# sipposip/pr-disagg-radar-gan

Measured on AMD Instinct MI355X. Metric: cWGAN-GP train samples/sec, 24x16x16 tiles, bs=256, higher is better.
Workload: dtype f32; 1 GPU; ndomain=16, 24h, bs=256 fp32, 1 critic step + 1 gen step (BASELINE configs[1]); batch_per_gpu=256, global_batch=256, n_critic=1, parallelism=dp1, world=1, rccl_ranks_seen=1, weights=random init (RandomNormal 0.02 / glorot_uniform), dropout 0.25 active

## Files before the change

include/rdgan.h:

```cpp
#ifndef RDGAN_H
#define RDGAN_H
#include <stdint.h>
#ifdef __cplusplus
extern "C" {
#endif

typedef struct rdgan_handle rdgan_handle;

#define RDGAN_LATENT_DIM 100
#define RDGAN_NHOURS 24
#define RDGAN_LOSS_SLOTS 8

int rdgan_create(rdgan_handle** out, int ndomain, int n_cond_channels, int max_batch);
void rdgan_destroy(rdgan_handle* h);
const char* rdgan_last_error(const rdgan_handle* h);
long rdgan_gen_param_count(const rdgan_handle* h);
long rdgan_critic_param_count(const rdgan_handle* h);
long rdgan_workspace_bytes(const rdgan_handle* h);

int rdgan_gen_forward(rdgan_handle* h, const float* gen_params, const float* z, const float* cond,
                      float* out, int B, void* stream);

int rdgan_check_numerics(rdgan_handle* h, void* stream);

int rdgan_critic_forward(rdgan_handle* h, const float* critic_params, const float* sample,
                         const float* cond, float* out, int B, uint64_t seed, void* stream);

int rdgan_critic_grad(rdgan_handle* h, const float* critic_params, const float* gen_params,
                      const float* x_real, const float* cond, const float* z, uint64_t seed,
                      float* grad_out, int B, void* stream);

int rdgan_critic_grad_after(rdgan_handle* h, const float* critic_params, const float* gen_params,
                            const float* x_real, const float* cond, const float* z, uint64_t seed,
                            float* grad_out, int B, void* critic_ready_event, void* stream);

int rdgan_gen_grad(rdgan_handle* h, const float* critic_params, const float* gen_params,
                   const float* z, const float* cond, uint64_t seed, float* grad_out, int B,
                   void* stream);

int rdgan_gen_grad_after(rdgan_handle* h, const float* critic_params, const float* gen_params,
                         const float* z, const float* cond, uint64_t seed, float* grad_out, int B,
                         void* critic_ready_event, void* stream);

int rdgan_adam(float* params, const float* grad, float* v, long n, int t, float lr, float beta2,
               float eps, float grad_scale, void* stream);

int rdgan_set_weight_versions(rdgan_handle* h, uint64_t gen_version, uint64_t critic_version);
int rdgan_form_builds(const rdgan_handle* h, long* gen_builds, long* critic_builds);

int rdgan_gen_param_layout(const rdgan_handle* h, long* offsets, long* sizes);
int rdgan_critic_param_layout(const rdgan_handle* h, long* offsets, long* sizes);

int rdgan_set_option(rdgan_handle* h, const char* name, int value);

enum {
  RDGAN_TAG_GCONV_FWD = 0,
  RDGAN_TAG_GCONV_DGRAD = 1,
// ... 87 lines not shown
```

pr_disagg_radar_gan_amd/_lib.py:

```python
import ctypes
import os

_HERE = os.path.dirname(os.path.abspath(__file__))
LIB_PATH = os.path.join(_HERE, "librdgan_hip.so")

c_f32p = ctypes.c_void_p
c_stream = ctypes.c_void_p

class LaunchStat(ctypes.Structure):
    _fields_ = [("plan", ctypes.c_int), ("kind", ctypes.c_int), ("batch", ctypes.c_int), ("launches", ctypes.c_int),
                ("gflop", ctypes.c_double), ("ms", ctypes.c_double), ("name", ctypes.c_char * 48), ("kernel", ctypes.c_char * 48)]


SIGNATURES = {
    "rdgan_create": (ctypes.c_int, [ctypes.POINTER(ctypes.c_void_p), ctypes.c_int, ctypes.c_int, ctypes.c_int]),
    "rdgan_destroy": (None, [ctypes.c_void_p]),
    "rdgan_last_error": (ctypes.c_char_p, [ctypes.c_void_p]),
    "rdgan_gen_param_count": (ctypes.c_long, [ctypes.c_void_p]),
    "rdgan_critic_param_count": (ctypes.c_long, [ctypes.c_void_p]),
    "rdgan_workspace_bytes": (ctypes.c_long, [ctypes.c_void_p]),
    "rdgan_gen_forward": (ctypes.c_int, [ctypes.c_void_p, c_f32p, c_f32p, c_f32p, c_f32p, ctypes.c_int, c_stream]),
    "rdgan_check_numerics": (ctypes.c_int, [ctypes.c_void_p, c_stream]),
    "rdgan_critic_forward": (ctypes.c_int, [ctypes.c_void_p, c_f32p, c_f32p, c_f32p, c_f32p, ctypes.c_int,
                                            ctypes.c_uint64, c_stream]),
    "rdgan_critic_grad": (ctypes.c_int, [ctypes.c_void_p, c_f32p, c_f32p, c_f32p, c_f32p, c_f32p, ctypes.c_uint64,
                                         c_f32p, ctypes.c_int, c_stream]),
    "rdgan_gen_grad": (ctypes.c_int, [ctypes.c_void_p, c_f32p, c_f32p, c_f32p, c_f32p, ctypes.c_uint64, c_f32p,
                                      ctypes.c_int, c_stream]),
    "rdgan_critic_grad_after": (ctypes.c_int, [ctypes.c_void_p, c_f32p, c_f32p, c_f32p, c_f32p, c_f32p, ctypes.c_uint64,
                                               c_f32p, ctypes.c_int, ctypes.c_void_p, c_stream]),
    "rdgan_gen_grad_after": (ctypes.c_int, [ctypes.c_void_p, c_f32p, c_f32p, c_f32p, c_f32p, ctypes.c_uint64, c_f32p,
                                            ctypes.c_int, ctypes.c_void_p, c_stream]),
    "rdgan_adam": (ctypes.c_int, [c_f32p, c_f32p, c_f32p, ctypes.c_long, ctypes.c_int, ctypes.c_float, ctypes.c_float,
                                  ctypes.c_float, ctypes.c_float, c_stream]),
    "rdgan_set_weight_versions": (ctypes.c_int, [ctypes.c_void_p, ctypes.c_uint64, ctypes.c_uint64]),
    "rdgan_form_builds": (ctypes.c_int, [ctypes.c_void_p, ctypes.POINTER(ctypes.c_long), ctypes.POINTER(ctypes.c_long)]),
    "rdgan_gen_param_layout": (ctypes.c_int, [ctypes.c_void_p, ctypes.POINTER(ctypes.c_long), ctypes.POINTER(ctypes.c_long)]),
    "rdgan_critic_param_layout": (ctypes.c_int, [ctypes.c_void_p, ctypes.POINTER(ctypes.c_long), ctypes.POINTER(ctypes.c_long)]),
    "rdgan_set_option": (ctypes.c_int, [ctypes.c_void_p, ctypes.c_char_p, ctypes.c_int]),
    "rdgan_profile": (ctypes.c_int, [ctypes.c_void_p, ctypes.c_uint]),
    "rdgan_flop_count": (ctypes.c_int, [ctypes.c_void_p, ctypes.POINTER(ctypes.c_double), ctypes.c_int]),
    "rdgan_profile_read": (ctypes.c_int, [ctypes.c_void_p, ctypes.c_int, ctypes.POINTER(ctypes.c_double),
                                          ctypes.POINTER(ctypes.c_long)]),
    "rdgan_profile_launches": (ctypes.c_int, [ctypes.c_void_p, ctypes.c_int]),
    "rdgan_launch_table": (ctypes.c_int, [ctypes.c_void_p, ctypes.POINTER(LaunchStat), ctypes.c_int, ctypes.POINTER(ctypes.c_int)]),
    "rdgan_data_gather": (ctypes.c_int, [c_f32p, ctypes.c_int, ctypes.c_int, ctypes.c_int, ctypes.c_void_p, ctypes.c_int,
                                         ctypes.c_int, ctypes.c_float, c_f32p, c_f32p, ctypes.c_void_p, c_stream]),
    "rdgan_data_valid_tiles": (ctypes.c_int, [c_f32p, ctypes.c_int, ctypes.c_int, ctypes.c_int, ctypes.c_int, ctypes.c_int,
                                              ctypes.c_float, ctypes.c_int, ctypes.c_void_p, c_stream]),
    "rdgan_crps_ensemble": (ctypes.c_int, [c_f32p, c_f32p, c_f32p, c_f32p, ctypes.c_int, ctypes.c_long, c_stream]),
    "rdgan_spectra_bins": (ctypes.c_int, [ctypes.c_int]),
    "rdgan_radial_spectra": (ctypes.c_int, [c_f32p, c_f32p, ctypes.c_long, ctypes.c_int, ctypes.c_int, c_stream]),
    "rdgan_lsd_workspace_bytes": (ctypes.c_long, [ctypes.c_long, ctypes.c_long]),
# ... 74 lines not shown
```

pr_disagg_radar_gan_amd/csrc/rdgan_api.hip:

```cpp
#include <hip/hip_runtime.h>
#include <stdio.h>
#include <string.h>
#include <math.h>
#include <string>
#include <vector>
#include <algorithm>
#include <unordered_set>

#include "../../include/rdgan.h"
#include "rdgan_plan.h"
#include "rdgan_hostplan.h"
#include "rdgan_rng.h"
#include "rdgan_gemm.hip.h"
#include "rdgan_gemm_ws.hip.h"
#include "rdgan_gemm_ws16.hip.h"
#include "rdgan_gemm_f16.hip.h"
#include "rdgan_upconv16.hip.h"
#include "rdgan_upconv16b.hip.h"
#include "rdgan_upconv16t.hip.h"
#include "rdgan_elem.hip.h"
#include "rdgan_data.hip.h"
#include "rdgan_edge.hip.h"
#include "rdgan_d2slab16.hip.h"
#include "rdgan_d2fwd16.hip.h"
// ... 70 lines not shown
  int collapse = 1;
  int tapgather = 1;
  int ws_ksplit = 1;
  int wave_spec = 1;
  int resident = 1;
  int edge_kernels = 1;
  int sample_offset = 0;
  float* g9b_tmp;
  float* gp_part;
  float* dw6_part;
  int side_on = 1;
  int split3 = 0;
  int dense_slices = 0;
  uint64_t gver_in = 0, cver_in = 0;
  const float* gcache_ptr = nullptr; uint64_t gcache_ver = 0; int gcache_cfg = -1;
  const float* ccache_ptr = nullptr; uint64_t ccache_ver = 0; int ccache_cfg = -1;
  long form_builds[2] = {0, 0};
  int keep_gates = 0;
  void* gate_keep[5] = {nullptr, nullptr, nullptr, nullptr, nullptr};
  int gate_keep_B = 0;
  hipStream_t side = nullptr;
  hipEvent_t ev_fork = nullptr, ev_join = nullptr, ev_cw = nullptr, ev_g[4] = {nullptr, nullptr, nullptr, nullptr};
  int* d_flag;
  std::unordered_set<const void*> lds_attr_done;
  int prof_launches = 0;
  std::vector<RdLaunchRec> launch_recs;
  size_t launch_used = 0;
  char cur_kernel[48] = {0};
  double flops_acc = 0;
  unsigned prof_mask = 0;
  std::vector<hipEvent_t> ev_start[RDGAN_NUM_TAGS], ev_stop[RDGAN_NUM_TAGS];
  size_t ev_used[RDGAN_NUM_TAGS] = {0};
};

#define RD_CHECK(h, call)                                                        \
  do {                                                                           \
    hipError_t e_ = (call);                                                      \
    if (e_ != hipSuccess) {                                                      \
      char b_[512];                                                              \
      snprintf(b_, sizeof b_, "%s:%d %s -> %s", __FILE__, __LINE__, #call, hipGetErrorString(e_)); \
      if (h) (h)->err = b_;                                                      \
      return (int)e_;                                                            \
    }                                                                            \
  } while (0)
#define RD_TRY(expr)            \
  do {                          \
// ... 665 lines not shown
    carve(h->h1, MB * h->gpix[1] * 256); carve(h->r1, MB * h->gpix[1]);
    carve(h->h2, MB * h->gpix[2] * 128); carve(h->r2, MB * h->gpix[2]);
    carve(h->h3, MB * h->gpix[3] * 64); carve(h->r3, MB * h->gpix[3]);
    carve(h->P9, MB * h->gpix[3] * 32);
    carve(h->fake, MB * h->gpix[3]);
    carve(h->dl, MB * h->gpix[3]);
    carve(h->gh3, MB * h->gpix[3] * 64);
    carve(h->gup3, MB * h->gpix[3] * 128);
    carve(h->dy2, MB * h->gpix[2] * 128);
    carve(h->gup2, MB * h->gpix[2] * 256);
    carve(h->dy1, MB * h->gpix[1] * 256);
    carve(h->gup1, MB * h->gpix[1] * 256);
    carve(h->ga0, MB * h->gpix[0] * 256);
    carve(h->cin, NB * h->dL[0] * h->CP);
    h->dh[0] = nullptr; h->du[0] = nullptr;
    for (int l = 1; l <= 4; ++l) { carve(h->dh[l], NB * h->dL[l] * dch[l]); carve(h->du[l], NB * h->dL[l] * dch[l]); }
    carve(h->v, NB);
    carve(h->P1, MB * h->dL[1] * h->ldp1);
    carve(h->g0, MB * h->dL[0]);
    carve(h->gpv, MB);
    carve(h->wpartial, h->wpartial_cap);
    carve(h->cpartial, h->cpartial_cap);
    carve(h->kpartial, h->kpartial_cap);
    h->DWT[0] = h->DWT[1] = nullptr;
    for (int l = 2; l <= 4; ++l) carve(h->DWT[l], 27L * dch[l - 1] * dch[l]);
    carve(h->W1T, 64 * h->ldp1);
    carve(h->W1P, 27L * h->CP * 64); carve(h->dW1P, 27L * h->CP * 64);
    h->GWT[0] = nullptr;
    for (int l = 1; l <= 3; ++l) carve(h->GWT[l], 27L * gch[l - 1] * gch[l]);
    carve(h->W9T, 64 * 32);
    h->GWC[0] = h->GWD[0] = nullptr;
    for (int l = 1; l <= 3; ++l) { carve(h->GWC[l], 64L * gch[l - 1] * gch[l]); carve(h->GWD[l], 64L * gch[l - 1] * gch[l]); }
    carve(h->dWc, 64L * 256 * 256);
    {
      size_t ne = 0, ns = 0;
      for (int l = 1; l <= 3; ++l) {
        const int* sd = h->gdim[l - 1];
        ne = std::max(ne, (size_t)(sd[0] + 1) * sd[1] * sd[2] * gch[l - 1]);
        ns = std::max(ns, (size_t)sd[0] * 4 * sd[1] * sd[2] * gch[l]);
      }
      h->fE[0] = h->fU[0] = nullptr;
      for (int l = 1; l <= 3; ++l) {
        const int* sd = h->gdim[l - 1];
        carve(h->fE[l], MB * (size_t)(sd[0] + 1) * sd[1] * sd[2] * gch[l - 1]);
        carve(h->fU[l], 48L * gch[l - 1] * gch[l]);
      }
// ... 12 lines not shown
          carve(p, 27L * dch[l - 1] * dch[l] / 2 + 8); h->bWB[l] = p;
        }
        h->bG1F[0] = nullptr;
        for (int l = 1; l <= 3; ++l) { carve(p, 32L * gch[l - 1] * gch[l] + 8); h->bG1F[l] = p; }
        carve(p, 32L * 256 * 256 + 8); h->bG1B = p;
        h->fWF[0] = h->fWF[1] = h->fWB[0] = h->fWB[1] = h->fG1F[0] = nullptr;
        for (int l = 2; l <= 4; ++l) {
          carve(p, 27L * dch[l - 1] * dch[l] / 2 + 8); h->fWF[l] = p;
          carve(p, 27L * dch[l - 1] * dch[l] / 2 + 8); h->fWB[l] = p;
        }
        for (int l = 1; l <= 3; ++l) { carve(p, 32L * gch[l - 1] * gch[l] + 8); h->fG1F[l] = p; }
        carve(p, 32L * 256 * 256 + 8); h->fG1B = p;
        carve(p, 32L * h->ldp1 + 8); h->bW1B = p;
        carve(p, 64L * 8 * 2 * 64 * 4 + 8); h->bW3I = p;
        carve(p, 64L * 8 * 2 * 64 * 4 + 8); h->bW3T = p;
        carve(p, 4L * 64 * 4 + 8); h->bW9I = p;
        carve(p, (long)RD_UP2_KSTEPS * 4 * 64 * 4 + 8); h->bW2I = p;
        carve(p, (long)RD_D2S_KSTEPS * 2 * 64 * 4 + 8); h->bW2S = p;
        if (nd % 16 == 0) { carve(p, NB * h->dL[1] * 4 + 8); if (pass == 1) h->g1bits = (unsigned char*)p; }
        carve(p, (long)RD_D2F_KSTEPS * 4 * 64 * 4 + 8); h->bW2F = p;
      }
      carve(h->fdU, 48L * 256 * 256); carve(h->fUT, 48L * 256 * 256);
    }
    { float* f = nullptr; carve(f, 64); if (pass == 1) h->d_flag = (int*)f; }
    carve(h->g9b_tmp, 64);
    carve(h->ubias_part, 32 * 8 * 64);
    carve(h->gp_part, (size_t)MB * 64);
    carve(h->dw6_part, (size_t)16 * h->F);
    if (pass == 0) {
      h->ws_bytes = off + 256;
      e = hipMalloc((void**)&h->ws, h->ws_bytes);
      if (e != hipSuccess) { (void)hipFree(h->d_plans); delete h; return (int)e; }
      (void)hipMemset(h->ws, 0, h->ws_bytes);
    }
  }
  {
    bool ok = hipStreamCreateWithFlags(&h->side, hipStreamNonBlocking) == hipSuccess;
    hipEvent_t* evs[] = {&h->ev_fork, &h->ev_join, &h->ev_cw, &h->ev_g[1], &h->ev_g[2], &h->ev_g[3]};
    for (hipEvent_t* e2 : evs) ok = ok && hipEventCreateWithFlags(e2, hipEventDisableTiming) == hipSuccess;
    if (!ok) { h->side_on = 0; (void)hipGetLastError(); }
  }
  *out = h;
  return 0;
}

extern "C" void rdgan_destroy(rdgan_handle* h) {
  if (!h) return;
  if (h->side) { (void)hipStreamSynchronize(h->side); (void)hipStreamDestroy(h->side); }
  for (hipEvent_t e2 : {h->ev_fork, h->ev_join, h->ev_cw, h->ev_g[1], h->ev_g[2], h->ev_g[3]}) if (e2) (void)hipEventDestroy(e2);
  for (auto& r : h->launch_recs) { (void)hipEventDestroy(r.e0); (void)hipEventDestroy(r.e1); }
  for (int t = 0; t < RDGAN_NUM_TAGS; ++t) {
    for (auto e : h->ev_start[t]) (void)hipEventDestroy(e);
    for (auto e : h->ev_stop[t]) (void)hipEventDestroy(e);
  }
  for (void* g : h->gate_keep) if (g) (void)hipFree(g);
  if (h->ws) (void)hipFree(h->ws);
  if (h->d_plans) (void)hipFree(h->d_plans);
  if (h->d_tab) (void)hipFree(h->d_tab);
  delete h;
}

extern "C" const char* rdgan_last_error(const rdgan_handle* h) { return h ? h->err.c_str() : "null handle"; }
extern "C" long rdgan_gen_param_count(const rdgan_handle* h) { return h ? h->n_gen : -1; }
extern "C" long rdgan_critic_param_count(const rdgan_handle* h) { return h ? h->n_critic : -1; }
extern "C" long rdgan_workspace_bytes(const rdgan_handle* h) { return h ? (long)h->ws_bytes : -1; }
extern "C" int rdgan_gen_param_layout(const rdgan_handle* h, long* offsets, long* sizes) {
  if (!h) return -2;
  for (int i = 0; i < 10; ++i) { if (offsets) offsets[i] = h->goff[i]; if (sizes) sizes[i] = h->gsz[i]; }
  return 10;
}
extern "C" int rdgan_critic_param_layout(const rdgan_handle* h, long* offsets, long* sizes) {
  if (!h) return -2;
// ... 24 lines not shown
  if (!strcmp(name, "d3_wgrad_slab")) { h->d3_wgrad_slab = value ? 1 : 0; return 0; }
  if (!strcmp(name, "d2_wgrad_slab")) { h->d2_wgrad_slab = value ? 1 : 0; return 0; }
  if (!strcmp(name, "upwgrad_slab")) { h->upwgrad_slab = value ? 1 : 0; return 0; }
  if (!strcmp(name, "d1_dgrad_fused")) { h->d1_dgrad_fused = value ? 1 : 0; return 0; }
  if (!strcmp(name, "d1_wgrad16")) { h->d1_wgrad16 = value ? 1 : 0; return 0; }
  if (!strcmp(name, "wgrad_wide")) { h->wgrad_wide = value ? 1 : 0; return 0; }
  if (!strcmp(name, "conv_f16")) {
    if (value < 0 || value > 2) return bad_arg(h, "conv_f16: 0, 1 or 2 (2: regardless of the launch size)");
    h->conv_f16 = value; h->ccache_ver = 0; h->gcache_ver = 0; return 0;
  }
  if (!strcmp(name, "d2_fwd_slab")) { h->d2_fwd_slab = value ? 1 : 0; h->ccache_ver = 0; return 0; }
  if (!strcmp(name, "d2_gate_bits")) { h->d2_gate_bits = value ? 1 : 0; return 0; }
  if (!strcmp(name, "d2_slab")) { h->d2_slab = value ? 1 : 0; h->ccache_ver = 0; return 0; }
  if (!strcmp(name, "dense_wgrad_slices")) { h->dense_slices = value; return 0; }
  if (!strcmp(name, "keep_gates")) {
    h->keep_gates = value ? 1 : 0;
    h->gate_keep_B = 0;
    for (int l = 1; l <= 4 && h->keep_gates; ++l)
      if (!h->gate_keep[l]) RD_CHECK(h, hipMalloc(&h->gate_keep[l], (size_t)h->MB * h->dL[l] * h->dch[l] * sizeof(float)));
    return 0;
  }
  if (!strcmp(name, "split3")) { h->split3 = value ? 1 : 0; return 0; }
  if (!strcmp(name, "side_stream")) { h->side_on = (value && h->side) ? 1 : 0; return 0; }
  if (!strcmp(name, "edge_kernels")) { h->edge_kernels = value < 0 ? 0 : (value > 2 ? 2 : value); return 0; }
  if (!strcmp(name, "sample_offset")) { if (value < 0) return bad_arg(h, "set_option: sample_offset < 0"); h->sample_offset = value; return 0; }
  if (!strcmp(name, "ws_ksplit")) { h->ws_ksplit = value < 0 ? 0 : (value > 8 ? 8 : value); return 0; }
  return bad_arg(h, "set_option: unknown option");
}

extern "C" int rdgan_set_weight_versions(rdgan_handle* h, uint64_t gen_version, uint64_t critic_version) {
  if (!h) return -2;
  h->gver_in = gen_version; h->cver_in = critic_version;
  return 0;
}
extern "C" int rdgan_form_builds(const rdgan_handle* h, long* gen_builds, long* critic_builds) {
  if (!h) return -2;
  if (gen_builds) *gen_builds = h->form_builds[0];
  if (critic_builds) *critic_builds = h->form_builds[1];
  return 0;
}

extern "C" int rdgan_profile(rdgan_handle* h, unsigned tag_mask) {
  if (!h) return -2;
  h->prof_mask = tag_mask;
  for (int t = 0; t < RDGAN_NUM_TAGS; ++t) {
    h->ev_used[t] = 0;
// ... 432 lines not shown
    RdEpi e = epi_make(RD_EPI_TAPGATHER);
    e.gw = nd; e.ghw = nd * nd; e.gq = gq;
    if (a16) RD_TRY(launch_conv_a16(h, h->plans[PL_G9F], h->d_plans + PL_G9F, B, h->h3, h->W9T, 32, h->P9, e, st, -1, true, false));
    else
    RD_TRY(launch_conv(h, h->plans[PL_G9F], h->d_plans + PL_G9F, B, h->h3, h->W9T, 32, h->P9, e, st, -1));
    ProfScope ps(h, RDGAN_TAG_ELEMENTWISE, st);
    if (gq == 3) hipLaunchKernelGGL((k_tapsum_softmax<RDGAN_NHOURS, 3>), dim3((unsigned)((ncol + 63) / 64)), dim3(256), 0, st, h->P9,
                                    gp + h->goff[9], out, B, nd, nd, h->d_flag);
    else hipLaunchKernelGGL((k_tapsum_softmax<RDGAN_NHOURS, 9>), dim3((unsigned)((ncol + 63) / 64)), dim3(256), 0, st, h->P9,
                            gp + h->goff[9], out, B, nd, nd, h->d_flag);
  } else {
    if (a16) RD_TRY(launch_conv_a16(h, h->plans[PL_G9F], h->d_plans + PL_G9F, B, h->h3, h->W9T, 32, h->P9, epi_make(RD_EPI_PLAIN), st, -1,
                                    true, false));
    else
    RD_TRY(launch_conv(h, h->plans[PL_G9F], h->d_plans + PL_G9F, B, h->h3, h->W9T, 32, h->P9, epi_make(RD_EPI_PLAIN), st, -1));
    ProfScope ps(h, RDGAN_TAG_ELEMENTWISE, st);
    hipLaunchKernelGGL(k_colgather_softmax, dim3((unsigned)((ncol + 63) / 64)), dim3(64), 0, st, h->P9, gp + h->goff[9],
                       out, B, RDGAN_NHOURS, nd, nd, h->d_flag);
  }
  RD_CHECK(h, hipGetLastError());
  return 0;
}

extern "C" int rdgan_gen_forward(rdgan_handle* h, const float* gen_params, const float* z, const float* cond,
                                 float* out, int B, void* stream) {
  if (!h || !gen_params || !z || !cond || !out) return bad_arg(h, "gen_forward: null pointer");
  if (B < 1 || B > h->MB) return bad_arg(h, "gen_forward: B outside [1, max_batch]");
  return gen_forward_impl(h, gen_params, z, cond, out, B, (hipStream_t)stream, side_fork(h, (hipStream_t)stream));
}

extern "C" int rdgan_check_numerics(rdgan_handle* h, void* stream) {
  if (!h) return -2;
  RD_CHECK(h, hipStreamSynchronize((hipStream_t)stream));
  int flag = 0;
  RD_CHECK(h, hipMemcpy(&flag, h->d_flag, sizeof(int), hipMemcpyDeviceToHost));
  if (flag) { h->err = "check_numerics: the generator output contains NaN or Inf"; return -1; }
  return 0;
}

static bool d2_slab_on(const rdgan_handle* h) { return h->d2_slab && h->a16 && h->nd == 16; }
static bool d2_slab_t_on(const rdgan_handle* h) {
  return h->d2_slab && h->a16 && h->nd > 16 && h->nd % 16 == 0 && h->ddim[2][1] % 4 == 0 && h->ddim[2][2] % 4 == 0 && h->ddim[2][0] == 6 &&
         h->ddim[1][1] == 2 * h->ddim[2][1] - 1 && h->ddim[1][2] == 2 * h->ddim[2][2] - 1 && h->dpad[1][0] == 1 && h->dpad[1][1] == 1 && h->dpad[1][2] == 1;
}
static bool d2_fwd_slab_on(const rdgan_handle* h) { return h->d2_fwd_slab && h->a16 && h->nd == 16; }
static int prep_critic_weights(rdgan_handle* h, const float* dp, hipStream_t st) {
  const int ccfg = (h->a16 ? 1 : 0) | (h->d2_slab ? 2 : 0) | (h->d2_fwd_slab ? 4 : 0);
  if (h->cver_in != 0 && dp == h->ccache_ptr && h->cver_in == h->ccache_ver && ccfg == h->ccache_cfg) return 0;
  h->form_builds[1]++;
  h->ccache_ptr = nullptr; h->ccache_ver = 0; h->ccache_cfg = -1;
// ... 224 lines not shown
    hipLaunchKernelGGL(k_d1_dgrad_tile16, dim3((unsigned)std::min<long>(items, 1024)), dim3(256), RD_D1DT_LDS, st, (const rd_bf16_t*)u1,
                       dp + h->doff[0], h->g0, B, h->nd);
    RD_CHECK(h, hipGetLastError());
    return 0;
  }
  if (h->a16)
    RD_TRY(launch_conv16(h, h->plans[PL_D1B], h->d_plans + PL_D1B, B, u1, h->bW1B, h->P1, epi_make(RD_EPI_PLAIN), st,
                         RDGAN_TAG_CRITIC_GEMM));
  else
  RD_TRY(launch_conv(h, h->plans[PL_D1B], h->d_plans + PL_D1B, B, u1, h->W1T, h->ldp1, h->P1, epi_make(RD_EPI_PLAIN), st,
                     RDGAN_TAG_CRITIC_GEMM));
  ProfScope ps(h, RDGAN_TAG_ELEMENTWISE, st);
  hipLaunchKernelGGL(k_d1_col2im, dim3(ew_blocks((long)B * h->dL[0])), dim3(256), 0, st, h->P1, h->g0, B, h->ddim[0][0],
                     h->ddim[0][1], h->ddim[0][2], h->ddim[1][0], h->ddim[1][1], h->ddim[1][2], h->Cin, h->ldp1);
  RD_CHECK(h, hipGetLastError());
  return 0;
}

extern "C" int rdgan_critic_forward(rdgan_handle* h, const float* critic_params, const float* sample, const float* cond,
                                    float* out, int B, uint64_t seed, void* stream) {
  if (!h || !critic_params || !sample || !cond || !out) return bad_arg(h, "critic_forward: null pointer");
  if (B < 1 || B > h->NB) return bad_arg(h, "critic_forward: B outside [1, 3*max_batch]");
  hipStream_t st = (hipStream_t)stream;
  h->gate_keep_B = 0;
  RD_TRY(a16_check(h));
  if (h->a16) RD_TRY(prep_critic_weights(h, critic_params, st));
  else if (h->CP != h->Cin && !(h->cver_in != 0 && critic_params == h->ccache_ptr && h->cver_in == h->ccache_ver)) {
    hipLaunchKernelGGL(k_pad_w1, dim3(27), dim3(256), 0, st, critic_params + h->doff[0], h->W1P, h->Cin, h->CP);
    h->ccache_ptr = nullptr; h->ccache_ver = 0; h->ccache_cfg = -1;
  }
  launch_build_critic_input(h, sample, nullptr, cond, B, 2, 0u, 0u, st);
  RD_TRY(critic_forward_impl(h, critic_params, B, seed, st));
  RD_CHECK(h, hipMemcpyAsync(out, h->v, sizeof(float) * B, hipMemcpyDeviceToDevice, st));
  return 0;
}

extern "C" int rdgan_critic_grad(rdgan_handle* h, const float* dp, const float* gp, const float* x_real,
                                 const float* cond, const float* z, uint64_t seed, float* grad, int B, void* stream) {
  return rdgan_critic_grad_after(h, dp, gp, x_real, cond, z, seed, grad, B, nullptr, stream);
}

extern "C" int rdgan_critic_grad_after(rdgan_handle* h, const float* dp, const float* gp, const float* x_real,
                                       const float* cond, const float* z, uint64_t seed, float* grad, int B,
                                       void* critic_ready_event, void* stream) {
  if (!h || !dp || !gp || !x_real || !cond || !z || !grad) return bad_arg(h, "critic_grad: null pointer");
  if (B < 1 || B > h->MB) return bad_arg(h, "critic_grad: B outside [1, max_batch]");
  hipStream_t st = (hipStream_t)stream;
  const int NBt = 3 * B;
  const int use_drop = seed != 0;
  hipStream_t ws = side_fork(h, st);
  RD_TRY(gen_forward_impl(h, gp, z, cond, h->fake, B, st, ws, false));
  if (critic_ready_event) RD_CHECK(h, hipStreamWaitEvent(ws, (hipEvent_t)critic_ready_event, 0));
  RD_TRY(prep_critic_weights(h, dp, ws));
  RD_TRY(side_join(h, st, h->ev_cw));
  const bool a16 = h->a16 != 0;
  {
    ProfScope ps(h, RDGAN_TAG_ELEMENTWISE, st);
    launch_build_critic_input(h, x_real, h->fake, cond, B, 0, rd_make_key(seed, RD_STREAM_ALPHA), (uint32_t)h->sample_offset, st);
  }
  RD_TRY(critic_forward_impl(h, dp, NBt, seed, st));
  RD_TRY(critic_dgrad_chain(h, dp, NBt, B, 0, seed, st));
  {
    hipStream_t cs = side_fork(h, st);
    for (int l = 1; l <= 4; ++l) {
      if (l == 1 && d1_gemm_ok(h) && d1_wgrad16_on(h)) continue;
      RD_TRY(launch_colsum(h, h->du[l], (long)2 * B * h->dL[l], h->dch[l], grad + h->doff[2 * (l - 1) + 1], cs, h->a16 != 0));
    }
  }
  RD_TRY(critic_input_grad(h, dp, act_off(h, h->du[1], (long)2 * B * h->dL[1] * 64), B, st));
  float* cin_hat = h->cin + (long)2 * B * h->dL[0] * h->CP;
  {
    ProfScope ps(h, RDGAN_TAG_ELEMENTWISE, st);
    const int per = (int)h->dL[0];
    const int S = std::max(1, std::min({(1024 + B - 1) / B, per / 4096, 64}));
    if (S > 1) hipLaunchKernelGGL(k_gp_norm_part, dim3(B * S), dim3(256), 0, st, h->g0, h->gp_part, per, S);
    hipLaunchKernelGGL(k_gp_norm_r0, dim3(B * S), dim3(256), 0, st, h->g0, cin_hat, h->gpv, per, B, RD_GP_WEIGHT, h->CP, S, h->gp_part);
  }
  h->gate_keep_B = 0;
  if (h->keep_gates) {
    for (int l = 1; l <= 4; ++l) {
      const long third = (long)2 * B * h->dL[l] * h->dch[l];
      RD_CHECK(h, hipMemcpyAsync(h->gate_keep[l], act_off(h, h->dh[l], third), (size_t)(third / 2) * (a16 ? 2 : 4),
// ... 85 lines not shown
    float* dwo = RS > 1 ? h->dw6_part : grad + h->doff[8];
    const dim3 dg((h->F + 15) / 16, RS);
    if (a16) hipLaunchKernelGGL(k_critic_dense_wgrad<rd_bf16_t>, dg, dim3(256), 0, st, (const rd_bf16_t*)h->dh[4], dwo, NBt, h->F, B);
    else hipLaunchKernelGGL(k_critic_dense_wgrad<float>, dg, dim3(256), 0, st, (const float*)h->dh[4], dwo, NBt, h->F, B);
    if (RS > 1) hipLaunchKernelGGL(k_reduce_partials, dim3((h->F + 15) / 16), dim3(256), 0, st, h->dw6_part, RS, h->F, grad + h->doff[8]);
    hipLaunchKernelGGL(k_critic_losses, dim3(1), dim3(256), 0, st, h->v, h->gpv, grad + h->n_critic, B, RD_GP_WEIGHT, h->d_flag,
                       grad + h->doff[9]);
  }
  RD_CHECK(h, hipGetLastError());
  return 0;
}

extern "C" int rdgan_gen_grad(rdgan_handle* h, const float* dp, const float* gp, const float* z, const float* cond,
                              uint64_t seed, float* grad, int B, void* stream) {
  return rdgan_gen_grad_after(h, dp, gp, z, cond, seed, grad, B, nullptr, stream);
}

extern "C" int rdgan_gen_grad_after(rdgan_handle* h, const float* dp, const float* gp, const float* z, const float* cond,
                                    uint64_t seed, float* grad, int B, void* critic_ready_event, void* stream) {
  if (!h || !dp || !gp || !z || !cond || !grad) return bad_arg(h, "gen_grad: null pointer");
  if (B < 1 || B > h->MB) return bad_arg(h, "gen_grad: B outside [1, max_batch]");
  hipStream_t st = (hipStream_t)stream;
  const int nd = h->nd;
  h->gate_keep_B = 0;
  if (!h->collapse)
    for (int l = 1; l <= 3; ++l)
      RD_TRY(launch_transpose(h, gp + h->goff[2 * l], h->GWT[l], 27, h->gch[l - 1], h->gch[l], h->gch[l - 1], st));
  hipStream_t ws = side_fork(h, st);
  RD_TRY(gen_forward_impl(h, gp, z, cond, h->fake, B, st, ws));
  if (critic_ready_event) RD_CHECK(h, hipStreamWaitEvent(ws, (hipEvent_t)critic_ready_event, 0));
  RD_TRY(prep_critic_weights(h, dp, ws));
  RD_TRY(side_join(h, st, h->ev_cw));
  {
    ProfScope ps(h, RDGAN_TAG_ELEMENTWISE, st);
    launch_build_critic_input(h, nullptr, h->fake, cond, B, 1, 0u, 0u, st);
  }
  RD_TRY(critic_forward_impl(h, dp, B, seed, st));
  RD_TRY(critic_dgrad_chain(h, dp, B, B, 1, seed, st));
  RD_TRY(critic_input_grad(h, dp, h->du[1], B, st));
  const bool a16 = h->a16 != 0;
  const long npix3 = (long)B * h->gpix[3];
  {
    ProfScope ps(h, RDGAN_TAG_ELEMENTWISE, st);
    long ncol = (long)B * nd * nd;
    hipLaunchKernelGGL(k_softmax_bwd, dim3((unsigned)((ncol + 63) / 64)), dim3(64), 0, st, h->fake, h->g0, h->dl, B,
                       RDGAN_NHOURS, nd, nd);
  }
  const size_t g9_lds = 4 * (size_t)(nd + 2) * (nd + 2) * sizeof(float);
  const bool g9_direct = h->g9_direct && g9_lds <= 96 * 1024 &&
                         (size_t)B * (RDGAN_NHOURS / 2) * 1728 <= h->wpartial_cap;
  if (a16 && !g9_direct) return bad_arg(h, "bf16 storage mode needs the direct backward of the last conv (g9_direct)");
  if (g9_direct) {
    ProfScope ps(h, RDGAN_TAG_GCONV_WGRAD, st);
    const size_t lds = std::max<size_t>(g9_lds, 4 * 27 * 16 * sizeof(f32x4));
    RD_TRY(ensure_lds(h, a16 ? (const void*)k_g9_bwd_pairs<rd_bf16_t> : (const void*)k_g9_bwd_pairs<float>, 96 * 1024));
// ... 729 lines not shown
    rc = (int)hipGetLastError();
  }
  if (rc == 0) rc = (int)hipStreamSynchronize(st);
  for (void* p : {xb, yb, wi, (void*)wc}) if (p) (void)hipFree(p);
  return rc;
}

extern "C" int rdgan_op_pixelnorm_lrelu(const float* y, float* hout, float* rinv, long npix, int C, void* stream) {
  if (!y || !hout) return -2;
  RD_TRY(launch_pn_fwd(nullptr, y, hout, rinv, npix, C, (hipStream_t)stream));
  return (int)hipStreamSynchronize((hipStream_t)stream);
}
extern "C" int rdgan_op_pixelnorm_lrelu_bwd(const float* gh, const float* hh, const float* rinv, float* dy, long npix, int C,
                                            void* stream) {
  if (!gh || !hh || !rinv || !dy) return -2;
  RD_TRY(launch_pn_bwd(nullptr, gh, hh, rinv, dy, npix, C, 0, 0, 0, 0, (hipStream_t)stream));
  return (int)hipStreamSynchronize((hipStream_t)stream);
}

__global__ void k_bytes_to_f32(const unsigned char* in, float* out, long n) {
  for (long i = blockIdx.x * (long)blockDim.x + threadIdx.x; i < n; i += (long)gridDim.x * blockDim.x) out[i] = (float)in[i];
}
extern "C" int rdgan_debug_activation(rdgan_handle* h, int which, float* out, long n, void* stream) {
  if (h && out && which == 8 && n >= 1) {
    if (!h->g1bits || n > (long)h->NB * h->dL[1] * 16) return bad_arg(h, "debug_activation: no gate bytes");
    hipLaunchKernelGGL(k_bytes_to_f32, dim3(ew_blocks(n)), dim3(256), 0, (hipStream_t)stream, h->g1bits, out, n);
    RD_CHECK(h, hipGetLastError());
    return 0;
  }
  if (!h || !out || which < 0 || which > 7 || n < 1) return bad_arg(h, "debug_activation: bad argument");
  const float* src; long cap;
  if (which < 4) {
    float* hs[4] = {h->h0, h->h1, h->h2, h->h3};
    src = hs[which]; cap = (long)h->MB * h->gpix[which] * h->gch[which];
  } else {
    const int l = which - 3;
    src = h->dh[l]; cap = (long)h->NB * h->dL[l] * h->dch[l];
  }
  if (n > cap) return bad_arg(h, "debug_activation: n exceeds the tensor");
  hipStream_t st = (hipStream_t)stream;
  auto copy = [&](const void* from, long first, long cnt) -> int {
    if (cnt <= 0) return 0;
    if (h->a16) {
      hipLaunchKernelGGL(k_bf16_to_f32, dim3(ew_blocks(cnt)), dim3(256), 0, st, (const rd_bf16_t*)from, out + first, cnt);
      RD_CHECK(h, hipGetLastError());
    } else
// ... 261 lines not shown
```

pr_disagg_radar_gan_amd/engine.py:

```python
import ctypes
import itertools

import numpy as np
import torch

from . import _lib
from . import weights as W

LOSS_SLOTS = 8

_versions = itertools.count(1)


def new_version():
    return next(_versions)


def require_gpu():
    if not torch.cuda.is_available():
        raise _lib.RdganError("no MI355X/ROCm device visible: the cWGAN-GP hot path runs only on the HIP "
                              "library (there is deliberately no CPU fallback)")


def _ptr(t):
# ... 78 lines not shown
    def check_numerics(self):
        rc = self.lib.rdgan_check_numerics(self._h, self._stream())
        if rc == -1:
            raise _lib.NumericsError("found nan in output of per_gridpoint_softmax")
        _lib.check(rc, self._h, "rdgan_check_numerics")

    def critic_forward(self, critic_params, sample, cond, seed=0, critic_version=0):
        B = sample.shape[0]
        nd = self.ndomain
        self._check_batch(B, 3 * self.max_batch)
        _chk_tensor(critic_params, (self.n_critic,), "critic_params")
        _chk_tensor(sample, (B, W.NHOURS, nd, nd, 1), "sample")
        _chk_tensor(cond, (B, nd, nd, self.n_cond_channels), "cond")
        out = torch.empty((B, 1), dtype=torch.float32, device=self.device)
        self._versions(0, critic_version)
        _lib.check(self.lib.rdgan_critic_forward(self._h, _ptr(critic_params), _ptr(sample), _ptr(cond), _ptr(out), B,
                                                 ctypes.c_uint64(seed), self._stream()), self._h, "rdgan_critic_forward")
        return out

    @staticmethod
    def _event_handle(ev):
        return ctypes.c_void_p(ev.cuda_event if ev is not None else 0)

    def critic_grad(self, critic_params, gen_params, x_real, cond, z, seed, grad_out=None, critic_ready=None,
                    gen_version=0, critic_version=0):
        B = x_real.shape[0]
        nd = self.ndomain
        self._check_batch(B, self.max_batch)
        _chk_tensor(critic_params, (self.n_critic,), "critic_params")
        _chk_tensor(gen_params, (self.n_gen,), "gen_params")
        _chk_tensor(x_real, (B, W.NHOURS, nd, nd, 1), "x_real")
        _chk_tensor(cond, (B, nd, nd, self.n_cond_channels), "cond")
        _chk_tensor(z, (B, W.LATENT_DIM), "z")
        if grad_out is None:
            grad_out = torch.empty(self.n_critic + LOSS_SLOTS, dtype=torch.float32, device=self.device)
        _chk_tensor(grad_out, (self.n_critic + LOSS_SLOTS,), "grad_out")
        self._versions(gen_version, critic_version)
        _lib.check(self.lib.rdgan_critic_grad_after(self._h, _ptr(critic_params), _ptr(gen_params), _ptr(x_real), _ptr(cond),
                                                    _ptr(z), ctypes.c_uint64(seed), _ptr(grad_out), B,
                                                    self._event_handle(critic_ready), self._stream()),
                   self._h, "rdgan_critic_grad")
        return grad_out

    def gen_grad(self, critic_params, gen_params, z, cond, seed, grad_out=None, critic_ready=None,
                 gen_version=0, critic_version=0):
        B = z.shape[0]
        nd = self.ndomain
        self._check_batch(B, self.max_batch)
        _chk_tensor(critic_params, (self.n_critic,), "critic_params")
        _chk_tensor(gen_params, (self.n_gen,), "gen_params")
        _chk_tensor(z, (B, W.LATENT_DIM), "z")
        _chk_tensor(cond, (B, nd, nd, self.n_cond_channels), "cond")
        if grad_out is None:
            grad_out = torch.empty(self.n_gen + LOSS_SLOTS, dtype=torch.float32, device=self.device)
        _chk_tensor(grad_out, (self.n_gen + LOSS_SLOTS,), "grad_out")
        self._versions(gen_version, critic_version)
        _lib.check(self.lib.rdgan_gen_grad_after(self._h, _ptr(critic_params), _ptr(gen_params), _ptr(z), _ptr(cond),
                                                 ctypes.c_uint64(seed), _ptr(grad_out), B,
                                                 self._event_handle(critic_ready), self._stream()),
                   self._h, "rdgan_gen_grad")
        return grad_out

    def adam(self, params, grad, v, t, lr=1e-4, beta2=0.9, eps=1e-7, grad_scale=1.0):
# ... 43 lines not shown
```

pr_disagg_radar_gan_amd/trainer.py:

```python
import numpy as np
import torch

LOSS_SLOTS = 8


SHARD_THRESHOLD_BYTES = 128 << 20


class WGANGPTrainer:

    def __init__(self, engine, gen_arrays, critic_arrays, n_disc=5, lr=1e-4, beta2=0.9, eps=1e-7,
                 process_group=None, world_size=1, rank=0, base_seed=1234, overlap=None, comm_hook=None, exchange=None,
                 grad_transport="fp32"):
        self.eng = engine
        self.n_disc = int(n_disc)
        self.lr, self.beta2, self.eps = lr, beta2, eps
        self.pg, self.world, self.rank = process_group, int(world_size), int(rank)
        if exchange not in (None, "auto", "allreduce", "sharded"):
            raise ValueError(f"exchange must be 'allreduce', 'sharded' or None, not {exchange!r}")
        if grad_transport not in ("fp32", "bf16"):
            raise ValueError(f"grad_transport must be 'fp32' or 'bf16', not {grad_transport!r}")
        self.grad_transport = grad_transport
        g0, d0 = engine.to_slab(gen_arrays), engine.to_slab(critic_arrays)
        self.exchange = {}
# ... 12 lines not shown
            grad = torch.zeros(max(P, n + LOSS_SLOTS), dtype=torch.float32, device=p0.device)
            setattr(self, which + "_pbuf", pbuf)
            setattr(self, which + "_vbuf", vbuf)
            setattr(self, which + "params", pbuf[:n])
            setattr(self, which + "v", vbuf[:n])
            setattr(self, which + "grad", grad[:n + LOSS_SLOTS] if not sharded else grad)
            if sharded:
                setattr(self, which + "_gshard", torch.zeros(per, dtype=torch.float32, device=p0.device))
                setattr(self, which + "_pshard", torch.zeros(per, dtype=torch.float32, device=p0.device))
        self.t = 0
        self.weight_cache = hasattr(engine, "form_builds")
        self.gver = self.dver = 0
        self.weights_changed()
        self.base_seed = int(base_seed)
        self.calls = 0
        on_gpu = self.gparams.is_cuda
        self.overlap = bool(on_gpu and (self.world > 1 if overlap is None else overlap))
        self.comm_hook = comm_hook
        self.comm = torch.cuda.Stream(device=self.gparams.device) if self.overlap else None
        self.d_ready = None
        self.g_ready = None
        self._native_collectives = None
        self._native_verified = set()

    def weights_changed(self, which="gd"):
        if self.weight_cache:
            from .engine import new_version
            for w in which:
                setattr(self, w + "ver", new_version())

    def _ver(self):
        return {"gen_version": self.gver, "critic_version": self.dver} if self.weight_cache else {}

    def _next_seed(self):
        self.calls += 1
        s = (self.base_seed * 0x9E3779B97F4A7C15 + self.calls * 0xD1B54A32D192ED03 + self.rank * 0x94D049BB133111EB)
        s &= 0xFFFFFFFFFFFFFFFF
        return s or 1

    def _allreduce(self, slab):
        if self.comm_hook is not None:
            self.comm_hook(slab)
        if self.world > 1:
            import torch.distributed as dist
            dist.all_reduce(slab, op=dist.ReduceOp.SUM, group=self.pg)

# ... 132 lines not shown

    def reduced_grad(self, which):
        n, per, P = self._pad[which]
        grad = getattr(self, which + "grad")
        self.join()
        if self.exchange[which] == "allreduce":
            return grad / self.world
        full = torch.empty(P, dtype=torch.float32, device=grad.device)
        self._all_gather(full, getattr(self, which + "_gshard"))
        return full / self.world

    def sync_state(self):
        self.join()
        for which in ("g", "d"):
            if self.exchange[which] == "sharded":
                n, per, P = self._pad[which]
                vbuf, psh = getattr(self, which + "_vbuf"), getattr(self, which + "_pshard")
                psh.copy_(vbuf[self.rank * per:(self.rank + 1) * per])
                self._all_gather(vbuf[:P], psh)

    def _slab(self, which):
        return getattr(self, which + "grad")[:self._pad[which][0] + LOSS_SLOTS]

    def critic_step(self, x_real, cond, z, seed=None):
        seed = self._next_seed() if seed is None else seed
        if not self.overlap:
            self.eng.critic_grad(self.dparams, self.gparams, x_real, cond, z, seed, grad_out=self._slab("d"), **self._ver())
            return self._update("d")
        cur = torch.cuda.current_stream(self.dparams.device)
        if self.g_ready is not None:
            cur.wait_event(self.g_ready)
        self.eng.critic_grad(self.dparams, self.gparams, x_real, cond, z, seed, grad_out=self._slab("d"), critic_ready=self.d_ready,
                             **self._ver())
        return self._update_overlapped("d")

    def gen_step(self, z, cond, seed=None):
        seed = self._next_seed() if seed is None else seed
        if not self.overlap:
            self.eng.gen_grad(self.dparams, self.gparams, z, cond, seed, grad_out=self._slab("g"), **self._ver())
            return self._update("g")
        cur = torch.cuda.current_stream(self.gparams.device)
        if self.g_ready is not None:
            cur.wait_event(self.g_ready)
        self.eng.gen_grad(self.dparams, self.gparams, z, cond, seed, grad_out=self._slab("g"), critic_ready=self.d_ready,
                          **self._ver())
        return self._update_overlapped("g")

    def join(self):
        if self.overlap:
            cur = torch.cuda.current_stream(self.gparams.device)
            for ev in (self.d_ready, self.g_ready):
                if ev is not None:
                    cur.wait_event(ev)

    def iteration_raw(self, critic_batches, gen_batch):
        assert len(critic_batches) == self.n_disc
        for (x, c, z) in critic_batches:
            dl = self.critic_step(x, c, z)
        gl = self.gen_step(*gen_batch)
        self.join()
        return dl, gl

    def iteration(self, critic_batches, gen_batch):
        assert len(critic_batches) == self.n_disc
        for (x, c, z) in critic_batches:
            dl = self.critic_step(x, c, z)
        gl = self.gen_step(*gen_batch)
        self.join()
        return 0.5 * (dl[1] + dl[2]), gl[0], torch.maximum(dl[4], gl[4])

    def state_arrays(self):
        from . import weights as W
        self.join()
        return (W.unflatten(self.gparams.cpu().numpy(), self.eng.gen_shapes),
                W.unflatten(self.dparams.cpu().numpy(), self.eng.critic_shapes))


    def save_checkpoint(self, path, extra=None, synced=False, write=True):
        st = np.random.get_state()
        if not synced:
            self.sync_state()
        if not write:
            return
        np.savez(path, format=np.array("rdgan-checkpoint-1"), ndomain=self.eng.ndomain,
                 n_cond_channels=getattr(self.eng, "n_cond_channels", 1),
                 gparams=self.gparams.cpu().numpy(), dparams=self.dparams.cpu().numpy(),
                 gv=self.gv.cpu().numpy(), dv=self.dv.cpu().numpy(),
                 t=self.t, calls=self.calls, base_seed=self.base_seed, n_disc=self.n_disc,
                 hyper=np.array([self.lr, self.beta2, self.eps], np.float64),
# ... 40 lines not shown
```

Baseline: 23320 samples/s.

## Run generator forward for gen step ahead on side stream during critic step

During the last critic step, the generator forward pass for the upcoming generator step is launched on a separate non-blocking stream. It writes its own copies of the partial buffers and flag, so it can overlap the critic forward and backward. gen_grad then skips recomputing the forward when params, inputs, batch and weight version match, and waits on the ahead event instead. This adds a stream, events and a duplicated workspace buffer. It risks hazards on the shared fake buffer, which critic_grad has already consumed into its critic input before the ahead forward is issued.

```diff
diff --git a/include/rdgan.h b/include/rdgan.h
--- a/include/rdgan.h
+++ b/include/rdgan.h
@@ -33,6 +33,11 @@
 int rdgan_critic_grad_after(rdgan_handle* h, const float* critic_params, const float* gen_params,
                             const float* x_real, const float* cond, const float* z, uint64_t seed,
                             float* grad_out, int B, void* critic_ready_event, void* stream);
+
+int rdgan_critic_grad_ahead(rdgan_handle* h, const float* critic_params, const float* gen_params,
+                            const float* x_real, const float* cond, const float* z, uint64_t seed,
+                            float* grad_out, int B, void* critic_ready_event, const float* gen_z, const float* gen_cond,
+                            int gen_B, void* stream);
 
 int rdgan_gen_grad(rdgan_handle* h, const float* critic_params, const float* gen_params,
                    const float* z, const float* cond, uint64_t seed, float* grad_out, int B,
diff --git a/pr_disagg_radar_gan_amd/_lib.py b/pr_disagg_radar_gan_amd/_lib.py
--- a/pr_disagg_radar_gan_amd/_lib.py
+++ b/pr_disagg_radar_gan_amd/_lib.py
@@ -29,6 +29,8 @@
                                       ctypes.c_int, c_stream]),
     "rdgan_critic_grad_after": (ctypes.c_int, [ctypes.c_void_p, c_f32p, c_f32p, c_f32p, c_f32p, c_f32p, ctypes.c_uint64,
                                                c_f32p, ctypes.c_int, ctypes.c_void_p, c_stream]),
+    "rdgan_critic_grad_ahead": (ctypes.c_int, [ctypes.c_void_p, c_f32p, c_f32p, c_f32p, c_f32p, c_f32p, ctypes.c_uint64,
+                                               c_f32p, ctypes.c_int, ctypes.c_void_p, c_f32p, c_f32p, ctypes.c_int, c_stream]),
     "rdgan_gen_grad_after": (ctypes.c_int, [ctypes.c_void_p, c_f32p, c_f32p, c_f32p, c_f32p, ctypes.c_uint64, c_f32p,
                                             ctypes.c_int, ctypes.c_void_p, c_stream]),
     "rdgan_adam": (ctypes.c_int, [c_f32p, c_f32p, c_f32p, ctypes.c_long, ctypes.c_int, ctypes.c_float, ctypes.c_float,
diff --git a/pr_disagg_radar_gan_amd/csrc/rdgan_api.hip b/pr_disagg_radar_gan_amd/csrc/rdgan_api.hip
--- a/pr_disagg_radar_gan_amd/csrc/rdgan_api.hip
+++ b/pr_disagg_radar_gan_amd/csrc/rdgan_api.hip
@@ -116,6 +116,15 @@
   hipStream_t side = nullptr;
   hipEvent_t ev_fork = nullptr, ev_join = nullptr, ev_cw = nullptr, ev_g[4] = {nullptr, nullptr, nullptr, nullptr};
   int* d_flag;
+  int fwd_ahead = -1;
+  hipStream_t ahead = nullptr;
+  hipEvent_t ev_ahead_fork = nullptr, ev_ahead_done = nullptr;
+  float* kpartial_ahead = nullptr;
+  int* flag_ahead = nullptr;
+  bool ahead_pending = false;
+  const float *ahead_gp = nullptr, *ahead_z = nullptr, *ahead_cond = nullptr;
+  int ahead_B = 0;
+  uint64_t ahead_gver = 0;
   std::unordered_set<const void*> lds_attr_done;
   int prof_launches = 0;
   std::vector<RdLaunchRec> launch_recs;
@@ -827,6 +836,7 @@
     carve(h->wpartial, h->wpartial_cap);
     carve(h->cpartial, h->cpartial_cap);
     carve(h->kpartial, h->kpartial_cap);
+    carve(h->kpartial_ahead, h->kpartial_cap);
     h->DWT[0] = h->DWT[1] = nullptr;
     for (int l = 2; l <= 4; ++l) carve(h->DWT[l], 27L * dch[l - 1] * dch[l]);
     carve(h->W1T, 64 * h->ldp1);
@@ -885,7 +895,7 @@
       }
       carve(h->fdU, 48L * 256 * 256); carve(h->fUT, 48L * 256 * 256);
     }
-    { float* f = nullptr; carve(f, 64); if (pass == 1) h->d_flag = (int*)f; }
+    { float* f = nullptr; carve(f, 64); if (pass == 1) { h->d_flag = (int*)f; h->flag_ahead = (int*)f + 32; } }
     carve(h->g9b_tmp, 64);
     carve(h->ubias_part, 32 * 8 * 64);
     carve(h->gp_part, (size_t)MB * 64);
@@ -902,6 +912,10 @@
     hipEvent_t* evs[] = {&h->ev_fork, &h->ev_join, &h->ev_cw, &h->ev_g[1], &h->ev_g[2], &h->ev_g[3]};
     for (hipEvent_t* e2 : evs) ok = ok && hipEventCreateWithFlags(e2, hipEventDisableTiming) == hipSuccess;
     if (!ok) { h->side_on = 0; (void)hipGetLastError(); }
+    bool ok2 = hipStreamCreateWithFlags(&h->ahead, hipStreamNonBlocking) == hipSuccess;
+    ok2 = ok2 && hipEventCreateWithFlags(&h->ev_ahead_fork, hipEventDisableTiming) == hipSuccess;
+    ok2 = ok2 && hipEventCreateWithFlags(&h->ev_ahead_done, hipEventDisableTiming) == hipSuccess;
+    if (!ok2) { h->ahead = nullptr; (void)hipGetLastError(); }
   }
   *out = h;
   return 0;
@@ -910,7 +924,9 @@
 extern "C" void rdgan_destroy(rdgan_handle* h) {
   if (!h) return;
   if (h->side) { (void)hipStreamSynchronize(h->side); (void)hipStreamDestroy(h->side); }
-  for (hipEvent_t e2 : {h->ev_fork, h->ev_join, h->ev_cw, h->ev_g[1], h->ev_g[2], h->ev_g[3]}) if (e2) (void)hipEventDestroy(e2);
+  if (h->ahead) { (void)hipStreamSynchronize(h->ahead); (void)hipStreamDestroy(h->ahead); }
+  for (hipEvent_t e2 : {h->ev_fork, h->ev_join, h->ev_cw, h->ev_g[1], h->ev_g[2], h->ev_g[3], h->ev_ahead_fork, h->ev_ahead_done})
+    if (e2) (void)hipEventDestroy(e2);
   for (auto& r : h->launch_recs) { (void)hipEventDestroy(r.e0); (void)hipEventDestroy(r.e1); }
   for (int t = 0; t < RDGAN_NUM_TAGS; ++t) {
     for (auto e : h->ev_start[t]) (void)hipEventDestroy(e);
@@ -981,6 +997,7 @@
   }
   if (!strcmp(name, "split3")) { h->split3 = value ? 1 : 0; return 0; }
   if (!strcmp(name, "side_stream")) { h->side_on = (value && h->side) ? 1 : 0; return 0; }
+  if (!strcmp(name, "gen_fwd_ahead")) { h->fwd_ahead = value < 0 ? -1 : (value ? 1 : 0); return 0; }
   if (!strcmp(name, "edge_kernels")) { h->edge_kernels = value < 0 ? 0 : (value > 2 ? 2 : value); return 0; }
   if (!strcmp(name, "sample_offset")) { if (value < 0) return bad_arg(h, "set_option: sample_offset < 0"); h->sample_offset = value; return 0; }
   if (!strcmp(name, "ws_ksplit")) { h->ws_ksplit = value < 0 ? 0 : (value > 8 ? 8 : value); return 0; }
@@ -1459,10 +1476,35 @@
   return 0;
 }
 
+static bool fwd_ahead_on(const rdgan_handle* h) { return h->ahead && h->ev_ahead_done && (h->fwd_ahead < 0 ? !h->a16 : h->fwd_ahead); }
+
+static int ahead_drain(rdgan_handle* h, hipStream_t st) {
+  if (!h->ahead_pending) return 0;
+  h->ahead_pending = false;
+  RD_CHECK(h, hipStreamWaitEvent(st, h->ev_ahead_done, 0));
+  return 0;
+}
+
+static int ahead_issue(rdgan_handle* h, const float* gp, const float* z, const float* cond, int B, hipStream_t st) {
+  RD_CHECK(h, hipEventRecord(h->ev_ahead_fork, st));
+  RD_CHECK(h, hipStreamWaitEvent(h->ahead, h->ev_ahead_fork, 0));
+  std::swap(h->kpartial, h->kpartial_ahead);
+  std::swap(h->d_flag, h->flag_ahead);
+  const int rc = gen_forward_impl(h, gp, z, cond, h->fake, B, h->ahead, h->ahead);
+  std::swap(h->kpartial, h->kpartial_ahead);
+  std::swap(h->d_flag, h->flag_ahead);
+  RD_TRY(rc);
+  RD_CHECK(h, hipEventRecord(h->ev_ahead_done, h->ahead));
+  h->ahead_pending = true;
+  h->ahead_gp = gp; h->ahead_z = z; h->ahead_cond = cond; h->ahead_B = B; h->ahead_gver = h->gver_in;
+  return 0;
+}
+
 extern "C" int rdgan_gen_forward(rdgan_handle* h, const float* gen_params, const float* z, const float* cond,
                                  float* out, int B, void* stream) {
   if (!h || !gen_params || !z || !cond || !out) return bad_arg(h, "gen_forward: null pointer");
   if (B < 1 || B > h->MB) return bad_arg(h, "gen_forward: B outside [1, max_batch]");
+  RD_TRY(ahead_drain(h, (hipStream_t)stream));
   return gen_forward_impl(h, gen_params, z, cond, out, B, (hipStream_t)stream, side_fork(h, (hipStream_t)stream));
 }
 
@@ -1733,6 +1775,7 @@
   if (!h || !critic_params || !sample || !cond || !out) return bad_arg(h, "critic_forward: null pointer");
   if (B < 1 || B > h->NB) return bad_arg(h, "critic_forward: B outside [1, 3*max_batch]");
   hipStream_t st = (hipStream_t)stream;
+  RD_TRY(ahead_drain(h, st));
   h->gate_keep_B = 0;
   RD_TRY(a16_check(h));
   if (h->a16) RD_TRY(prep_critic_weights(h, critic_params, st));
@@ -1754,9 +1797,19 @@
 extern "C" int rdgan_critic_grad_after(rdgan_handle* h, const float* dp, const float* gp, const float* x_real,
                                        const float* cond, const float* z, uint64_t seed, float* grad, int B,
                                        void* critic_ready_event, void* stream) {
+  return rdgan_critic_grad_ahead(h, dp, gp, x_real, cond, z, seed, grad, B, critic_ready_event, nullptr, nullptr, 0, stream);
+}
+
+extern "C" int rdgan_critic_grad_ahead(rdgan_handle* h, const float* dp, const float* gp, const float* x_real,
+                                       const float* cond, const float* z, uint64_t seed, float* grad, int B,
+                                       void* critic_ready_event, const float* gen_z, const float* gen_cond, int gen_B,
+                                       void* stream) {
   if (!h || !dp || !gp || !x_real || !cond || !z || !grad) return bad_arg(h, "critic_grad: null pointer");
   if (B < 1 || B > h->MB) return bad_arg(h, "critic_grad: B outside [1, max_batch]");
+  if ((gen_z != nullptr) != (gen_cond != nullptr)) return bad_arg(h, "critic_grad: gen_z and gen_cond go together");
+  if (gen_z && (gen_B < 1 || gen_B > h->MB)) return bad_arg(h, "critic_grad: gen_B outside [1, max_batch]");
   hipStream_t st = (hipStream_t)stream;
+  RD_TRY(ahead_drain(h, st));
   const int NBt = 3 * B;
   const int use_drop = seed != 0;
   hipStream_t ws = side_fork(h, st);
@@ -1769,6 +1822,7 @@
     ProfScope ps(h, RDGAN_TAG_ELEMENTWISE, st);
     launch_build_critic_input(h, x_real, h->fake, cond, B, 0, rd_make_key(seed, RD_STREAM_ALPHA), (uint32_t)h->sample_offset, st);
   }
+  if (gen_z && fwd_ahead_on(h)) RD_TRY(ahead_issue(h, gp, gen_z, gen_cond, gen_B, st));
   RD_TRY(critic_forward_impl(h, dp, NBt, seed, st));
   RD_TRY(critic_dgrad_chain(h, dp, NBt, B, 0, seed, st));
   {
@@ -1900,15 +1954,23 @@
   if (B < 1 || B > h->MB) return bad_arg(h, "gen_grad: B outside [1, max_batch]");
   hipStream_t st = (hipStream_t)stream;
   const int nd = h->nd;
+  const bool ahead = h->ahead_pending && gp == h->ahead_gp && z == h->ahead_z && cond == h->ahead_cond && B == h->ahead_B &&
+                     h->gver_in == h->ahead_gver;
+  if (!ahead) RD_TRY(ahead_drain(h, st));
+  h->ahead_pending = false;
   h->gate_keep_B = 0;
   if (!h->collapse)
     for (int l = 1; l <= 3; ++l)
       RD_TRY(launch_transpose(h, gp + h->goff[2 * l], h->GWT[l], 27, h->gch[l - 1], h->gch[l], h->gch[l - 1], st));
   hipStream_t ws = side_fork(h, st);
-  RD_TRY(gen_forward_impl(h, gp, z, cond, h->fake, B, st, ws));
+  if (!ahead) RD_TRY(gen_forward_impl(h, gp, z, cond, h->fake, B, st, ws));
   if (critic_ready_event) RD_CHECK(h, hipStreamWaitEvent(ws, (hipEvent_t)critic_ready_event, 0));
   RD_TRY(prep_critic_weights(h, dp, ws));
   RD_TRY(side_join(h, st, h->ev_cw));
+  if (ahead) {
+    RD_CHECK(h, hipStreamWaitEvent(st, h->ev_ahead_done, 0));
+    std::swap(h->d_flag, h->flag_ahead);
+  }
   {
     ProfScope ps(h, RDGAN_TAG_ELEMENTWISE, st);
     launch_build_critic_input(h, nullptr, h->fake, cond, B, 1, 0u, 0u, st);
@@ -2684,6 +2746,7 @@
   for (long i = blockIdx.x * (long)blockDim.x + threadIdx.x; i < n; i += (long)gridDim.x * blockDim.x) out[i] = (float)in[i];
 }
 extern "C" int rdgan_debug_activation(rdgan_handle* h, int which, float* out, long n, void* stream) {
+  if (h) RD_TRY(ahead_drain(h, (hipStream_t)stream));
   if (h && out && which == 8 && n >= 1) {
     if (!h->g1bits || n > (long)h->NB * h->dL[1] * 16) return bad_arg(h, "debug_activation: no gate bytes");
     hipLaunchKernelGGL(k_bytes_to_f32, dim3(ew_blocks(n)), dim3(256), 0, (hipStream_t)stream, h->g1bits, out, n);
diff --git a/pr_disagg_radar_gan_amd/engine.py b/pr_disagg_radar_gan_amd/engine.py
--- a/pr_disagg_radar_gan_amd/engine.py
+++ b/pr_disagg_radar_gan_amd/engine.py
@@ -124,8 +124,10 @@
     def _event_handle(ev):
         return ctypes.c_void_p(ev.cuda_event if ev is not None else 0)
 
+    forward_ahead = True
+
     def critic_grad(self, critic_params, gen_params, x_real, cond, z, seed, grad_out=None, critic_ready=None,
-                    gen_version=0, critic_version=0):
+                    gen_version=0, critic_version=0, gen_batch=None):
         B = x_real.shape[0]
         nd = self.ndomain
         self._check_batch(B, self.max_batch)
@@ -137,10 +139,20 @@
         if grad_out is None:
             grad_out = torch.empty(self.n_critic + LOSS_SLOTS, dtype=torch.float32, device=self.device)
         _chk_tensor(grad_out, (self.n_critic + LOSS_SLOTS,), "grad_out")
+        gz = gc = None
+        gB = 0
+        if gen_batch is not None:
+            gz, gc = gen_batch
+            gB = gz.shape[0]
+            self._check_batch(gB, self.max_batch)
+            _chk_tensor(gz, (gB, W.LATENT_DIM), "gen_batch z")
+            _chk_tensor(gc, (gB, nd, nd, self.n_cond_channels), "gen_batch cond")
         self._versions(gen_version, critic_version)
-        _lib.check(self.lib.rdgan_critic_grad_after(self._h, _ptr(critic_params), _ptr(gen_params), _ptr(x_real), _ptr(cond),
+        _lib.check(self.lib.rdgan_critic_grad_ahead(self._h, _ptr(critic_params), _ptr(gen_params), _ptr(x_real), _ptr(cond),
                                                     _ptr(z), ctypes.c_uint64(seed), _ptr(grad_out), B,
-                                                    self._event_handle(critic_ready), self._stream()),
+                                                    self._event_handle(critic_ready),
+                                                    ctypes.c_void_p(gz.data_ptr() if gz is not None else 0),
+                                                    ctypes.c_void_p(gc.data_ptr() if gc is not None else 0), gB, self._stream()),
                    self._h, "rdgan_critic_grad")
         return grad_out
 
diff --git a/pr_disagg_radar_gan_amd/trainer.py b/pr_disagg_radar_gan_amd/trainer.py
--- a/pr_disagg_radar_gan_amd/trainer.py
+++ b/pr_disagg_radar_gan_amd/trainer.py
@@ -58,6 +58,7 @@
         self.g_ready = None
         self._native_collectives = None
         self._native_verified = set()
+        self._gen_batch_next = None
 
     def weights_changed(self, which="gd"):
         if self.weight_cache:
@@ -236,16 +237,21 @@
     def _slab(self, which):
         return getattr(self, which + "grad")[:self._pad[which][0] + LOSS_SLOTS]
 
-    def critic_step(self, x_real, cond, z, seed=None):
+    def critic_step(self, x_real, cond, z, seed=None, gen_batch=None):
         seed = self._next_seed() if seed is None else seed
+        if gen_batch is None:
+            gen_batch, self._gen_batch_next = self._gen_batch_next, None
+        kw = self._ver()
+        if gen_batch is not None and getattr(self.eng, "forward_ahead", False):
+            kw["gen_batch"] = tuple(gen_batch)
         if not self.overlap:
-            self.eng.critic_grad(self.dparams, self.gparams, x_real, cond, z, seed, grad_out=self._slab("d"), **self._ver())
+            self.eng.critic_grad(self.dparams, self.gparams, x_real, cond, z, seed, grad_out=self._slab("d"), **kw)
             return self._update("d")
         cur = torch.cuda.current_stream(self.dparams.device)
         if self.g_ready is not None:
             cur.wait_event(self.g_ready)
         self.eng.critic_grad(self.dparams, self.gparams, x_real, cond, z, seed, grad_out=self._slab("d"), critic_ready=self.d_ready,
-                             **self._ver())
+                             **kw)
         return self._update_overlapped("d")
 
     def gen_step(self, z, cond, seed=None):
@@ -269,16 +275,20 @@
 
     def iteration_raw(self, critic_batches, gen_batch):
         assert len(critic_batches) == self.n_disc
-        for (x, c, z) in critic_batches:
+        for k, (x, c, z) in enumerate(critic_batches):
+            self._gen_batch_next = gen_batch if k == self.n_disc - 1 else None
             dl = self.critic_step(x, c, z)
+        self._gen_batch_next = None
         gl = self.gen_step(*gen_batch)
         self.join()
         return dl, gl
 
     def iteration(self, critic_batches, gen_batch):
         assert len(critic_batches) == self.n_disc
-        for (x, c, z) in critic_batches:
+        for k, (x, c, z) in enumerate(critic_batches):
+            self._gen_batch_next = gen_batch if k == self.n_disc - 1 else None
             dl = self.critic_step(x, c, z)
+        self._gen_batch_next = None
         gl = self.gen_step(*gen_batch)
         self.join()
         return 0.5 * (dl[1] + dl[2]), gl[0], torch.maximum(dl[4], gl[4])
```

Result: faster. 23860 samples/s, median of 6 (+2.3%).
